# NVlabs/FoundationPose

Hardware: NVIDIA H100
Metric: pose-hypotheses/sec at 640x480 RGB-D, 252 hyp, 5 refine iters (higher is better)
Workload: dtype f16

## Files before the change

### foundationpose_b200/csrc/fp_api_ops.cu

```cuda
#include "../../include/fpose.h"
#include "fp_common.cuh"
#include "fp_attn.cuh"
#include "fp_crop.cuh"
#include "fp_gemm.cuh"

#include <vector>

namespace fp {
const char* get_last_error();
int prof_collect(int kind, double* total_ms, double* total_work, int* launches);
}

extern "C" {

const char* fp_last_error(void) { return fp::get_last_error(); }

unsigned long long fp_launch_count(void) { return fp::launch_count(); }

int fp_prof_enable(int on) {
  fp::g_prof_on = on != 0;
  return 0;
}

int fp_prof_collect(int kind, double* total_ms, double* total_work, int* launches) {
  if (!total_ms || !total_work || !launches) {
    fp::set_last_error("fp_prof_collect: null output");
    return -1;
  }
  return fp::prof_collect(kind, total_ms, total_work, launches);
}

int fp_op_build_meshlets(int V, int F, const float* pos, const int* faces, int* info, int* face_of_tri_out,
                         float* meshlets_out) {
  try {
    if (!pos || !faces || !info || V <= 0 || F <= 0) {
      fp::set_last_error("fp_op_build_meshlets: bad argument");
      return -1;
    }
    for (int i = 0; i < 3 * F; ++i)
      if (faces[i] < 0 || faces[i] >= V) {
        fp::set_last_error("fp_op_build_meshlets: face index out of range");
        return -1;
      }
    std::vector<float> nrm((size_t)V * 3, 0.f), att((size_t)V * 3, 0.f);
    fp::MeshHost mh;
    int rc = fp::build_mesh_host(V, F, pos, nrm.data(), att.data(), 3, faces, mh);
    if (rc) return rc;
    int max_t = 0, max_v = 0, total = 0;
    for (const fp::Meshlet& m : mh.meshlets) {
      max_t = m.n_tris > max_t ? m.n_tris : max_t;
      max_v = m.n_verts > max_v ? m.n_verts : max_v;
      total += m.n_tris;
      for (int t = 0; t < m.n_tris; ++t) {
        const uint2 tr = mh.ml_tris[m.tri_off + t];
        for (int k = 0; k < 3; ++k) {
          const int slot = (tr.x >> (8 * k)) & 255;
          if (slot >= m.n_verts || mh.ml_verts[m.vert_off + slot] != faces[3 * tr.y + k]) {
            fp::set_last_error("fp_op_build_meshlets: meshlet triangle does not map back to its face");
            return -4;
          }
          const float* q = pos + 3 * faces[3 * tr.y + k];
          const float dx = q[0] - m.cx, dy = q[1] - m.cy, dz = q[2] - m.cz;
          if (dx * dx + dy * dy + dz * dz > m.r * m.r * 1.0001f + 1e-12f) {
            fp::set_last_error("fp_op_build_meshlets: vertex outside the meshlet's bounding sphere");
            return -4;
          }
        }
        if (face_of_tri_out) face_of_tri_out[m.tri_off + t] = (int)tr.y;
      }
    }
    if (meshlets_out)
      for (size_t i = 0; i < mh.meshlets.size(); ++i) {
        const fp::Meshlet& m = mh.meshlets[i];
        const float rec[8] = {m.cx, m.cy, m.cz, m.r, m.ax, m.ay, m.az, m.cutoff};
        for (int k = 0; k < 8; ++k) meshlets_out[8 * i + k] = rec[k];
      }
    info[0] = (int)mh.meshlets.size();
    info[1] = mh.closed;
    info[2] = mh.front_sign;
    info[3] = max_t;
    info[4] = max_v;
    info[5] = total;
    return 0;
  } catch (...) {
    fp::set_last_error("fp_op_build_meshlets: exception");
    return -3;
  }
}

int fp_op_attention(const void* qkv, void* out, int B, int impl, void* stream) {
  if (!qkv || !out) {
    fp::set_last_error("fp_op_attention: null argument");
    return -1;
  }
  fp::AttnParams ap;
  ap.qkv = reinterpret_cast<const __half*>(qkv);
  ap.ld = 1536;
  ap.q_off = 0;
  ap.k_off = 512;
  ap.v_off = 1024;
  ap.group_col_stride = 0;
  ap.n_groups = 1;
  ap.out = reinterpret_cast<__half*>(out);
  ap.ld_out = 512;
  ap.out_group_stride = 0;
  ap.B = B;
  ap.T = 400;
  ap.n_heads = 4;
  ap.scale = 0.08838834764831845f;
  cudaStream_t st = reinterpret_cast<cudaStream_t>(stream);
  (void)impl;
  return fp::attn_tc_launch(ap, st);
}

static fp::GemmLayer to_gemm_layer(const fp_gemm_layer_t* l) {
  fp::GemmLayer L;
  L.kind = l->kind;
  L.n_img = l->n_img;
  L.Hin = l->Hin;
  L.Win = l->Win;
  L.Cin = l->Cin;
  L.Cout = l->Cout;
  L.in = l->in;
  L.w = l->w;
  L.bias = l->bias;
  L.res = l->res;
  L.res_ld = l->res_ld;
  L.out = l->out;
  L.out_ld = l->out_ld;
  L.out_split = l->out_split;
  L.post_add = l->post_add;
  L.relu = l->relu;
  return L;
}

int fp_op_gemm_layer(const fp_gemm_layer_t* l, void* stream) {
  if (!l) {
    fp::set_last_error("fp_op_gemm_layer: null layer");
    return -1;
  }
  return fp::gemm_layer_launch(to_gemm_layer(l), reinterpret_cast<cudaStream_t>(stream));
}

int fp_op_gemm_tile_n(const fp_gemm_layer_t* l, int* tile_n) {
  if (!l || !tile_n) {
    fp::set_last_error("fp_op_gemm_tile_n: null argument");
    return -1;
  }
  return fp::gemm_layer_tile_n(to_gemm_layer(l), tile_n);
}

}
```

### foundationpose_b200/csrc/fp_gemm.cu

```cuda
#include "fp_gemm.cuh"

#include <stdarg.h>
#include <stdlib.h>
#include <string.h>

#include <mutex>
#include <vector>

#include "fp_common.cuh"
#include "fp_wgmma.cuh"

namespace fp {

static std::atomic<unsigned long long> g_launch_count{0};
static thread_local bool t_capturing = false;
void note_launches(int n) {
  if (!t_capturing) g_launch_count.fetch_add((unsigned long long)n, std::memory_order_relaxed);
}
unsigned long long launch_count() { return g_launch_count.load(std::memory_order_relaxed); }
void set_capturing(bool on) { t_capturing = on; }

std::atomic<bool> g_prof_on{false};
static std::mutex g_prof_mu;

struct ProfRec {
  cudaEvent_t e0, e1;
  double work;
  int kind;
};
static std::vector<ProfRec> g_prof_recs;

void prof_mark_begin(int kind, double work, cudaStream_t stream) {
  if (!g_prof_on) return;
  ProfRec r;
  r.kind = kind;
  r.work = work;
  cudaEventCreate(&r.e0);
  cudaEventCreate(&r.e1);
  cudaEventRecord(r.e0, stream);
  std::lock_guard<std::mutex> lk(g_prof_mu);
  g_prof_recs.push_back(r);
}
void prof_mark_end(cudaStream_t stream) {
  if (!g_prof_on) return;
  std::lock_guard<std::mutex> lk(g_prof_mu);
  if (g_prof_recs.empty()) return;
  cudaEventRecord(g_prof_recs.back().e1, stream);
}
int prof_collect(int kind, double* total_ms, double* total_work, int* launches) {
  FP_CUDA_OK(cudaDeviceSynchronize());
  std::lock_guard<std::mutex> lk(g_prof_mu);
  double ms = 0, work = 0;
  int n = 0;
  std::vector<ProfRec> keep;
  for (auto& r : g_prof_recs) {
    if (r.kind != kind) {
      keep.push_back(r);
      continue;
    }
    float t = 0.f;
    cudaEventElapsedTime(&t, r.e0, r.e1);
    ms += t;
    work += r.work;
    ++n;
    cudaEventDestroy(r.e0);
    cudaEventDestroy(r.e1);
  }
  g_prof_recs.swap(keep);
  *total_ms = ms;
  *total_work = work;
  *launches = n;
  return 0;
}

static thread_local char t_last_error[1024] = "";
void set_last_error(const char* fmt, ...) {
  va_list ap;
  va_start(ap, fmt);
  vsnprintf(t_last_error, sizeof(t_last_error), fmt, ap);
  va_end(ap);
}
const char* get_last_error() { return t_last_error; }

static thread_local int t_pdl_skip = 0;
void pdl_skip_next() { t_pdl_skip = 1; }

bool pdl_enabled() {
  if (t_pdl_skip) {
    t_pdl_skip = 0;
    return false;
  }
  static int on = -1;
  if (on < 0) {
    const char* e = getenv("FPOSE_PDL");
    on = (e && e[0] == '0') ? 0 : 1;
  }
  return on != 0;
}

struct GemmParams {
  int lg_bw, lg_bh;
  int bw, bh, bn;
  int tiles_w, tiles_h, tiles_n, n_tiles_n, total_tiles;
  int num_kb, chunks_per_tap;
  int dim_w, dim_h, dim_n;
  short tap_off[9][5];
  int Ho, Wo, n_img, Cout;
  const float* bias;
  int has_res;
  int odim_h, odim_n;
  int out_split;
  const float* post_add;
  int relu;
  double alg_flops;
};

constexpr int kBlockM = 128;
constexpr int kBlockK = 64;
constexpr int kABytes = kBlockM * kBlockK * 2;
constexpr int kTileThreads = 384;
constexpr int kSlabBytes = kBlockM * 64 * 2;
constexpr int kSmemOptIn = 232448;

constexpr int kWideSlabs = 2;
constexpr int kWideProducerRegs = 40;
constexpr int kWideConsumerRegs = 232;
template <int BN>
struct TileCfg {
  static constexpr int kBBytes = BN * kBlockK * 2;
  static constexpr int kStageBytes = kABytes + kBBytes;
  static constexpr int kSlabs = BN > 128 ? kWideSlabs : BN / 64;
  static constexpr int kPasses = BN / 64 / kSlabs;
  static constexpr int kStagingBytes = kSlabs * kSlabBytes;
  static constexpr int kRing = kSmemOptIn - kStagingBytes - 1024  - 256 ;
  static constexpr int kStages = (kRing / kStageBytes) > 8 ? 8 : (kRing / kStageBytes);
  static constexpr int kSmemBytes = kStages * kStageBytes + kStagingBytes + 1024 + 256;
  static_assert(kSmemBytes <= kSmemOptIn, "tile configuration exceeds the 227 KB opt-in shared memory");
  static_assert(kPasses * kSlabs * 64 == BN, "the epilogue passes must cover the tile's channels");
};

template <int BN>
__global__ void __launch_bounds__(kTileThreads, 1)
    gemm_tile_kernel(const __grid_constant__ CUtensorMap map_a, const __grid_constant__ CUtensorMap map_b,
                     const __grid_constant__ CUtensorMap map_out, const __grid_constant__ CUtensorMap map_res,
                     const __grid_constant__ GemmParams p) {
  using Cfg = TileCfg<BN>;
  constexpr int S = Cfg::kStages;
  constexpr int NSLAB = Cfg::kSlabs;
  constexpr int JP = BN / 8 / Cfg::kPasses;
  extern __shared__ uint8_t smem_raw[];
  uint8_t* smem = reinterpret_cast<uint8_t*>((reinterpret_cast<uintptr_t>(smem_raw) + 1023) & ~uintptr_t(1023));
  uint8_t* staging = smem + S * Cfg::kStageBytes;
  uint64_t* bars = reinterpret_cast<uint64_t*>(staging + Cfg::kStagingBytes);
  uint64_t* full = bars;
  uint64_t* empty = bars + S;
  uint64_t* res_full = bars + 2 * S;

  const int m_tiles = p.tiles_w * p.tiles_h * p.tiles_n;
  const int total = m_tiles * p.n_tiles_n;

  if (threadIdx.x == 0) {
    tma_prefetch_desc(&map_a);
    tma_prefetch_desc(&map_b);
    tma_prefetch_desc(&map_out);
    if (p.has_res) tma_prefetch_desc(&map_res);
    for (int s = 0; s < S; ++s) {
      mbar_init(&full[s], 1);
      mbar_init(&empty[s], 256);
    }
    mbar_init(res_full, 1);
    mbar_fence_init();
  }
  __syncthreads();
  pdl_trigger();
  pdl_wait();

  auto decode = [&](int t, int& n_tile, int& tw, int& th, int& tn) {
    n_tile = t % p.n_tiles_n;
    const int m_tile = t / p.n_tiles_n;
    tw = m_tile % p.tiles_w;
    th = (m_tile / p.tiles_w) % p.tiles_h;
    tn = m_tile / (p.tiles_w * p.tiles_h);
  };

  if (threadIdx.x < 128) {
    if constexpr (BN > 128) regs_release<kWideProducerRegs>();
    if (threadIdx.x == 0) {
      int stage = 0, phase = 0;
      for (int t = blockIdx.x; t < total; t += gridDim.x) {
        int n_tile, tw, th, tn;
        decode(t, n_tile, tw, th, tn);
        int base[5] = {0, 0, 0, 0, 0};
        base[p.dim_w] += tw * p.bw;
        if (p.dim_h >= 0) base[p.dim_h] += th * p.bh;
        if (p.dim_n >= 0) base[p.dim_n] += tn * p.bn;
        int tap = 0, chunk = 0;
        for (int kb = 0; kb < p.num_kb; ++kb) {
          mbar_wait(&empty[stage], phase ^ 1);
          uint8_t* sa = smem + stage * Cfg::kStageBytes;
          mbar_expect_tx(&full[stage], Cfg::kStageBytes);
          tma_load_5d(&map_a, &full[stage], sa, base[0] + p.tap_off[tap][0] + chunk * kBlockK, base[1] + p.tap_off[tap][1],
                      base[2] + p.tap_off[tap][2], base[3] + p.tap_off[tap][3], base[4] + p.tap_off[tap][4]);
          tma_load_2d(&map_b, &full[stage], sa + kABytes, kb * kBlockK, n_tile * BN);
          if (++chunk == p.chunks_per_tap) {
            chunk = 0;
            ++tap;
          }
          if (++stage == S) {
            stage = 0;
            phase ^= 1;
          }
        }
      }
    }
    return;
  }

  if constexpr (BN > 128) regs_acquire<kWideConsumerRegs>();
  const int ct = threadIdx.x - 128;
  const int cw = ct >> 7;
  const int lane = threadIdx.x & 31;
  const int r0 = 64 * cw + 16 * ((ct >> 5) & 3) + (lane >> 2);
  const int cq = 2 * (lane & 3);
  const bool leader = (ct == 0);
  float acc[BN / 2];
#pragma unroll
  for (int i = 0; i < BN / 2; ++i) acc[i] = 0.f;
  int stage = 0, phase = 0, it = 0;
  for (int t = blockIdx.x; t < total; t += gridDim.x, ++it) {
    int n_tile, tw, th, tn;
    decode(t, n_tile, tw, th, tn);
    const int n0 = tn * p.bn;
    int n_o0 = n0, coff = 0;
    if (p.out_split > 0) {
      n_o0 = n0 % p.out_split;
      coff = (n0 / p.out_split) * p.Cout;
    }
    int oc[5] = {0, 0, 0, 0, 0}, rc[5] = {0, 0, 0, 0, 0};
    oc[1] = rc[1] = tw * p.bw;
    if (p.odim_h >= 0) oc[p.odim_h] = rc[p.odim_h] = th * p.bh;
    if (p.odim_n >= 0) {
      oc[p.odim_n] = n_o0;
      rc[p.odim_n] = n0;
    }
    if (leader) asm volatile("cp.async.bulk.wait_group.read 0;" ::: "memory");
    asm volatile("bar.sync 1, 256;" ::: "memory");
    if (leader && p.has_res) {
      mbar_expect_tx(res_full, NSLAB * kSlabBytes);
      for (int s = 0; s < NSLAB; ++s)
        tma_load_5d(&map_res, res_full, staging + s * kSlabBytes, n_tile * BN + s * 64, rc[1], rc[2], rc[3], rc[4]);
    }

    int prev = -1;
    for (int kb = 0; kb < p.num_kb; ++kb) {
      mbar_wait(&full[stage], phase);
      const uint32_t sa = smem_u32(smem + stage * Cfg::kStageBytes);
      const uint64_t da = gmma_desc_sw128(sa + (uint32_t)cw * 8192u);
      const uint64_t db = gmma_desc_sw128(sa + kABytes);
      wgmma_fence();
#pragma unroll
      for (int k = 0; k < kBlockK / 16; ++k)
        Wgmma<BN>::ss(acc, da + (uint64_t)(2 * k), db + (uint64_t)(2 * k), (kb > 0 || k > 0) ? 1u : 0u);
      wgmma_commit();
      if (prev >= 0) {
        wgmma_wait<1>();
        mbar_arrive(&empty[prev]);
      }
      prev = stage;
      if (++stage == S) {
        stage = 0;
        phase ^= 1;
      }
    }
    wgmma_wait<0>();
    fence_regs(acc);
    if (prev >= 0) mbar_arrive(&empty[prev]);

    const float* bias = p.bias + n_tile * BN;
    const float* pap[2] = {nullptr, nullptr};
    if (p.post_add) {
#pragma unroll
      for (int h = 0; h < 2; ++h) {
        const int row = r0 + 8 * h;
        const int jj = row & (p.bw - 1), ii = (row >> p.lg_bw) & (p.bh - 1);
        const int i = th * p.bh + ii, j = min(tw * p.bw + jj, p.Wo - 1);
        pap[h] = p.post_add + (size_t)(i * p.Wo + j) * p.Cout + n_tile * BN;
      }
    }
#pragma unroll
    for (int ps = 0; ps < Cfg::kPasses; ++ps) {
      const int c0 = n_tile * BN + ps * NSLAB * 64;
      if (ps > 0) {
        if (leader) asm volatile("cp.async.bulk.wait_group.read 0;" ::: "memory");
        asm volatile("bar.sync 1, 256;" ::: "memory");
        if (leader && p.has_res) {
          mbar_expect_tx(res_full, NSLAB * kSlabBytes);
          for (int s = 0; s < NSLAB; ++s)
            tma_load_5d(&map_res, res_full, staging + s * kSlabBytes, c0 + s * 64, rc[1], rc[2], rc[3], rc[4]);
        }
      }
      if (p.has_res) mbar_wait(res_full, (uint32_t)((it * Cfg::kPasses + ps) & 1));
#pragma unroll
      for (int jl = 0; jl < JP; ++jl) {
        const int j = ps * JP + jl;
        const int col = 8 * j + cq;
        const float2 b = __ldg(reinterpret_cast<const float2*>(bias + col));
        uint8_t* slab = staging + (jl >> 3) * kSlabBytes;
#pragma unroll
        for (int h = 0; h < 2; ++h) {
          const int row = r0 + 8 * h;
          uint32_t* cell = reinterpret_cast<uint32_t*>(slab + row * 128 + ((((uint32_t)j & 7u) ^ (uint32_t)(row & 7)) << 4) + cq * 2);
          float a0 = acc[4 * j + 2 * h] + b.x, a1 = acc[4 * j + 2 * h + 1] + b.y;
          if (p.has_res) {
            const float2 r = __half22float2(*reinterpret_cast<const __half2*>(cell));
            a0 += r.x;
            a1 += r.y;
          }
          if (p.relu) {
            a0 = fmaxf(a0, 0.f);
            a1 = fmaxf(a1, 0.f);
          }
          if (pap[h]) {
            const float2 pe = __ldg(reinterpret_cast<const float2*>(pap[h] + col));
            a0 += pe.x;
            a1 += pe.y;
          }
          *cell = pack_half2(a0, a1);
        }
      }
      asm volatile("fence.proxy.async.shared::cta;" ::: "memory");
      asm volatile("bar.sync 1, 256;" ::: "memory");
      if (leader) {
        for (int s = 0; s < NSLAB; ++s)
          tma_store_5d(&map_out, staging + s * kSlabBytes, coff + c0 + s * 64, oc[1], oc[2], oc[3], oc[4]);
        asm volatile("cp.async.bulk.commit_group;" ::: "memory");
      }
    }
  }
  if (leader) asm volatile("cp.async.bulk.wait_group 0;" ::: "memory");
}

static int g_num_sms = 0;

typedef CUresult (*EncodeTiledFn)(CUtensorMap*, CUtensorMapDataType, cuuint32_t, void*, const cuuint64_t*,
                                  const cuuint64_t*, const cuuint32_t*, const cuuint32_t*,
                                  CUtensorMapInterleave, CUtensorMapSwizzle, CUtensorMapL2promotion,
                                  CUtensorMapFloatOOBfill);

static EncodeTiledFn get_encode_fn() {
  static EncodeTiledFn fn = nullptr;
  static std::once_flag once;
  std::call_once(once, [] {
    void* p = nullptr;
    cudaDriverEntryPointQueryResult qres;
    if (cudaGetDriverEntryPoint("cuTensorMapEncodeTiled", &p, cudaEnableDefault, &qres) == cudaSuccess &&
        qres == cudaDriverEntryPointSuccess)
      fn = reinterpret_cast<EncodeTiledFn>(p);
  });
  return fn;
}

static int encode_map(CUtensorMap* map, const void* base, int rank, const uint64_t* dims,
                      const uint64_t* strides_bytes , const uint32_t* box, bool swizzle128 = true) {
  EncodeTiledFn fn = get_encode_fn();
  FP_REQUIRE(fn != nullptr, "cuTensorMapEncodeTiled entry point not available (no CUDA driver?)");
  cuuint64_t gdim[5];
  cuuint64_t gstr[4];
  cuuint32_t bdim[5];
  cuuint32_t estr[5];
  for (int i = 0; i < rank; ++i) {
    gdim[i] = dims[i];
    bdim[i] = box[i];
    estr[i] = 1;
  }
  for (int i = 0; i < rank - 1; ++i) gstr[i] = strides_bytes[i];
  CUresult r = fn(map, CU_TENSOR_MAP_DATA_TYPE_FLOAT16, (cuuint32_t)rank, const_cast<void*>(base), gdim, gstr,
                  bdim, estr, CU_TENSOR_MAP_INTERLEAVE_NONE, swizzle128 ? CU_TENSOR_MAP_SWIZZLE_128B : CU_TENSOR_MAP_SWIZZLE_NONE,
                  CU_TENSOR_MAP_L2_PROMOTION_L2_256B, CU_TENSOR_MAP_FLOAT_OOB_FILL_NONE);
  FP_REQUIRE(r == CUDA_SUCCESS,
             "cuTensorMapEncodeTiled failed (%d): rank %d dims [%llu %llu %llu %llu %llu] box [%u %u %u %u %u]",
             (int)r, rank, (unsigned long long)dims[0], (unsigned long long)(rank > 1 ? dims[1] : 0),
             (unsigned long long)(rank > 2 ? dims[2] : 0), (unsigned long long)(rank > 3 ? dims[3] : 0),
             (unsigned long long)(rank > 4 ? dims[4] : 0), box[0], rank > 1 ? box[1] : 0, rank > 2 ? box[2] : 0,
             rank > 3 ? box[3] : 0, rank > 4 ? box[4] : 0);
  return 0;
}

int encode_map_f16(CUtensorMap* map, const void* base, int rank, const uint64_t* dims, const uint64_t* strides_bytes,
                   const uint32_t* box) {
  return encode_map(map, base, rank, dims, strides_bytes, box);
}
int encode_map_f16_linear(CUtensorMap* map, const void* base, int rank, const uint64_t* dims,
                          const uint64_t* strides_bytes, const uint32_t* box) {
  return encode_map(map, base, rank, dims, strides_bytes, box, false);
}
int num_sms() {
  if (g_num_sms == 0) {
    int dev = 0;
    if (cudaGetDevice(&dev) != cudaSuccess) return 0;
    if (cudaDeviceGetAttribute(&g_num_sms, cudaDevAttrMultiProcessorCount, dev) != cudaSuccess) return 0;
  }
  return g_num_sms;
}

static int ilog2(int v) {
  int l = 0;
  while ((1 << l) < v) ++l;
  return l;
}

template <int BN>
static int launch_bn(const CUtensorMap& ma, const CUtensorMap& mb, const CUtensorMap& mo, const CUtensorMap& mr,
                     const GemmParams& p, cudaStream_t stream) {
  using Cfg = TileCfg<BN>;
  static std::atomic<unsigned long long> attr_mask{0};
  if (!device_bit_test(attr_mask)) {
    FP_CUDA_OK(cudaFuncSetAttribute(gemm_tile_kernel<BN>, cudaFuncAttributeMaxDynamicSharedMemorySize, Cfg::kSmemBytes));
    device_bit_set(attr_mask);
  }
  const int sms = num_sms();
  FP_REQUIRE(sms > 0, "no CUDA device");
  const int grid = p.total_tiles < sms ? p.total_tiles : sms;
  prof_mark_begin(0, p.alg_flops, stream);
  FP_CUDA_OK(launch_pdl(gemm_tile_kernel<BN>, dim3(grid), dim3(kTileThreads), Cfg::kSmemBytes, stream, 1, ma, mb, mo, mr, p));
  prof_mark_end(stream);
  note_launches(1);
  FP_CUDA_OK(cudaGetLastError());
  return 0;
}

int stem_conv_launch(const GemmLayer& L, cudaStream_t stream);

static int gemm_layer_plan(const GemmLayer& L, cudaStream_t stream, int* tile_n) {
  if (L.kind == LK_CONV7_S2) {
    if (tile_n) {
      *tile_n = 64;
      return 0;
    }
    return stem_conv_launch(L, stream);
  }
  GemmParams p;
  memset(&p, 0, sizeof(p));
  CUtensorMap ma, mb;
  const uint64_t E = 2;
  int Ho, Wo, taps, ktot;
  int BN;
  uint64_t dims[5], str[4];
  uint32_t box[5];

  switch (L.kind) {
    case LK_LINEAR: {
      FP_REQUIRE(L.Cin % 64 == 0, "LINEAR: K=%d not a multiple of 64", L.Cin);
      Ho = 1;
      Wo = L.Win;
      taps = 1;
      p.chunks_per_tap = L.Cin / 64;
      p.bw = 128; p.bh = 1; p.bn = 1;
      p.dim_w = 1; p.dim_h = -1; p.dim_n = -1;
      dims[0] = L.Cin; dims[1] = L.Win; dims[2] = 1; dims[3] = 1; dims[4] = 1;
      str[0] = L.Cin * E; str[1] = str[0] * L.Win; str[2] = str[1]; str[3] = str[1];
      box[0] = 64; box[1] = 128; box[2] = 1; box[3] = 1; box[4] = 1;
      p.tiles_w = (L.Win + 127) / 128; p.tiles_h = 1; p.tiles_n = 1;
      break;
    }
    case LK_CONV3_S1: {
      FP_REQUIRE(L.Cin % 64 == 0, "CONV3_S1: Cin=%d not a multiple of 64", L.Cin);
      Ho = L.Hin; Wo = L.Win;
      taps = 9;
      p.chunks_per_tap = L.Cin / 64;
      if (Wo % 8 == 0 && Ho % 8 == 0) { p.bw = 8; p.bh = 8; p.bn = 2; }
      else if (Wo % 4 == 0 && Ho % 4 == 0) { p.bw = 4; p.bh = 4; p.bn = 8; }
      else FP_REQUIRE(false, "CONV3_S1: unsupported spatial size %dx%d", Ho, Wo);
      const uint64_t sw_ = (uint64_t)L.Cin * E, sh_ = sw_ * L.Win, sn_ = sh_ * L.Hin;
      p.dim_w = 1; p.dim_h = 2; p.dim_n = 3;
      dims[0] = L.Cin; dims[1] = L.Win; dims[2] = L.Hin; dims[3] = L.n_img; dims[4] = 1;
      str[0] = sw_; str[1] = sh_; str[2] = sn_; str[3] = sn_ * L.n_img;
      box[0] = 64; box[1] = p.bw; box[2] = p.bh; box[3] = p.bn; box[4] = 1;
      for (int r = 0; r < 3; ++r)
        for (int s = 0; s < 3; ++s) {
          p.tap_off[r * 3 + s][1] = (short)(s - 1);
          p.tap_off[r * 3 + s][2] = (short)(r - 1);
        }
      p.tiles_w = Wo / p.bw; p.tiles_h = Ho / p.bh; p.tiles_n = (L.n_img + p.bn - 1) / p.bn;
      break;
    }
    case LK_CONV3_S2: {
      FP_REQUIRE(L.Cin % 64 == 0, "CONV3_S2: Cin=%d not a multiple of 64", L.Cin);
      FP_REQUIRE(L.Hin % 2 == 0 && L.Win % 2 == 0, "CONV3_S2: odd input size");
      Ho = L.Hin / 2; Wo = L.Win / 2;
      taps = 9;
      p.chunks_per_tap = L.Cin / 64;
      if (Wo % 8 == 0 && Ho % 8 == 0) { p.bw = 8; p.bh = 8; p.bn = 2; }
      else if (Wo % 4 == 0 && Ho % 4 == 0) { p.bw = 4; p.bh = 4; p.bn = 8; }
      else FP_REQUIRE(false, "CONV3_S2: unsupported output size %dx%d", Ho, Wo);
      p.dim_w = 1; p.dim_h = 3; p.dim_n = 4;
      dims[0] = 2 * L.Cin; dims[1] = Wo; dims[2] = 2; dims[3] = Ho; dims[4] = L.n_img;
      str[0] = 2 * L.Cin * E; str[1] = (uint64_t)L.Win * L.Cin * E; str[2] = 2 * str[1];
      str[3] = (uint64_t)L.Hin * L.Win * L.Cin * E;
      box[0] = 64; box[1] = p.bw; box[2] = 1; box[3] = p.bh; box[4] = p.bn;
      for (int r = 0; r < 3; ++r)
        for (int s = 0; s < 3; ++s) {
          const int t = r * 3 + s;
          p.tap_off[t][0] = (short)((s == 1 ? 0 : 1) * L.Cin);
          p.tap_off[t][1] = (short)(s == 0 ? -1 : 0);
          p.tap_off[t][2] = (short)(r == 1 ? 0 : 1);
          p.tap_off[t][3] = (short)(r == 0 ? -1 : 0);
        }
      p.tiles_w = Wo / p.bw; p.tiles_h = Ho / p.bh; p.tiles_n = (L.n_img + p.bn - 1) / p.bn;
      break;
    }
    default:
      FP_REQUIRE(false, "unknown layer kind %d", L.kind);
  }
  ktot = taps * L.Cin;
  p.num_kb = ktot / 64;
  p.lg_bw = ilog2(p.bw);
  p.lg_bh = ilog2(p.bh);

  constexpr int kWideMinWaves = 8;
  constexpr int kWideMinKBlocks = 16;
  const int m_tiles = p.tiles_w * p.tiles_h * p.tiles_n;
  if (L.Cout % 256 == 0 && p.num_kb >= kWideMinKBlocks) {
    const int sms = num_sms();
    FP_REQUIRE(sms > 0, "no CUDA device");
    BN = (long long)m_tiles * (L.Cout / 256) >= (long long)kWideMinWaves * sms ? 256 : 128;
  } else if (L.Cout % 128 == 0) BN = 128;
  else if (L.Cout % 64 == 0) BN = 64;
  else FP_REQUIRE(false, "Cout=%d must be a multiple of 64", L.Cout);
  p.n_tiles_n = L.Cout / BN;
  p.total_tiles = p.tiles_w * p.tiles_h * p.tiles_n * p.n_tiles_n;
  p.Ho = Ho; p.Wo = Wo; p.n_img = L.n_img; p.Cout = L.Cout;
  p.bias = L.bias;
  p.has_res = L.res != nullptr;
  p.out_split = L.out_split;
  p.post_add = L.post_add;
  p.relu = L.relu;
  {
    const double k_real = (double)taps * L.Cin;
    p.alg_flops = 2.0 * (double)L.n_img * Ho * Wo * L.Cout * k_real;
  }
  FP_REQUIRE(L.out_ld % 8 == 0 && (!L.res || L.res_ld % 8 == 0), "out_ld / res_ld must be multiples of 8");
  FP_REQUIRE(L.out_split == 0 || L.out_split % p.bn == 0,
             "out_split=%d must be a multiple of the tile's image count %d (pad the A/B batch boundary)", L.out_split,
             p.bn);
  if (tile_n) {
    *tile_n = BN;
    return 0;
  }
  if (p.total_tiles == 0) return 0;

  int rc = encode_map(&ma, L.in, 5, dims, str, box);
  if (rc) return rc;
  uint64_t wd[2] = {(uint64_t)ktot, (uint64_t)L.Cout};
  uint64_t ws[1] = {(uint64_t)ktot * E};
  uint32_t wb[2] = {64, (uint32_t)BN};
  rc = encode_map(&mb, L.w, 2, wd, ws, wb);
  if (rc) return rc;
  CUtensorMap mo, mr;
  {
    uint64_t od[5], os[4];
    uint32_t ob[5];
    const bool lin = (L.kind == LK_LINEAR);
    const int n_out = L.out_split > 0 ? (L.n_img - L.out_split) : L.n_img;
    FP_REQUIRE(n_out > 0, "out_split=%d leaves no output images (n_img=%d)", L.out_split, L.n_img);
    auto fill = [&](int ld, int nimg) {
      const uint64_t sw_ = (uint64_t)ld * E, sh_ = sw_ * Wo, sn_ = sh_ * Ho;
      od[0] = (uint64_t)ld;
      ob[0] = 64;
      od[4] = 1;
      ob[4] = 1;
      if (lin) {
        od[1] = (uint64_t)Wo; od[2] = 1; od[3] = 1;
        os[0] = sw_; os[1] = sh_; os[2] = sh_; os[3] = sh_;
        ob[1] = (uint32_t)p.bw; ob[2] = 1; ob[3] = 1;
      } else {
        od[1] = (uint64_t)Wo; od[2] = (uint64_t)Ho; od[3] = (uint64_t)nimg;
        os[0] = sw_; os[1] = sh_; os[2] = sn_; os[3] = sn_ * nimg;
        ob[1] = (uint32_t)p.bw; ob[2] = (uint32_t)p.bh; ob[3] = (uint32_t)p.bn;
      }
    };
    p.odim_h = lin ? -1 : 2;
    p.odim_n = lin ? -1 : 3;
    fill(L.out_ld, n_out);
    rc = encode_map(&mo, L.out, 5, od, os, ob);
    if (rc) return rc;
    if (L.res) {
      fill(L.res_ld, L.n_img);
      rc = encode_map(&mr, L.res, 5, od, os, ob);
      if (rc) return rc;
    } else {
      mr = mo;
    }
  }
  if (BN == 256) return launch_bn<256>(ma, mb, mo, mr, p, stream);
  return BN == 128 ? launch_bn<128>(ma, mb, mo, mr, p, stream) : launch_bn<64>(ma, mb, mo, mr, p, stream);
}

int gemm_layer_launch(const GemmLayer& L, cudaStream_t stream) { return gemm_layer_plan(L, stream, nullptr); }

int gemm_layer_tile_n(const GemmLayer& L, int* tile_n) { return gemm_layer_plan(L, nullptr, tile_n); }

}
```

### foundationpose_b200/csrc/fp_gemm.cuh

```cuda
#pragma once
#include <cuda.h>
#include <cuda_runtime.h>
#include <stdint.h>

#include <atomic>

namespace fp {

enum LayerKind : int {
  LK_LINEAR = 0,
  LK_CONV3_S1 = 1,
  LK_CONV3_S2 = 2,
  LK_CONV7_S2 = 3,
};

struct GemmLayer {
  int kind;
  int n_img;
  int Hin, Win;
  int Cin;
  int Cout;
  const void* in;
  const void* w;
  const float* bias;
  const void* res;
  int res_ld;
  void* out;
  int out_ld;
  int out_split;
  const float* post_add;
  int relu;
};

int gemm_layer_launch(const GemmLayer& L, cudaStream_t stream);
int gemm_layer_tile_n(const GemmLayer& L, int* tile_n);


void prof_mark_begin(int kind, double work, cudaStream_t stream);
void prof_mark_end(cudaStream_t stream);
extern std::atomic<bool> g_prof_on;

}
```

### foundationpose_b200/ops.py

```python
import ctypes as C

import torch

from . import _lib
from ._lib import lib


def _ptr(t):
    return None if t is None else C.c_void_p(t.data_ptr())


def _stream():
    return C.c_void_p(torch.cuda.current_stream().cuda_stream)


def _require_cuda(*ts):
    for t in ts:
        if t is not None and not t.is_cuda:
            raise _lib.FposeError("libfpose operators need CUDA tensors (there is no CPU path)")


def gemm_layer(kind, x, w_packed, bias, *, n_img, Hin, Win, Cin, Cout, out=None, out_ld=None, out_split=0,
               res=None, res_ld=0, post_add=None, relu=False):
    _require_cuda(x, w_packed, bias, res, post_add, out)
    assert x.dtype == torch.float16 and w_packed.dtype == torch.float16 and bias.dtype == torch.float32
    if kind == _lib.LAYER_LINEAR:
        Ho, Wo = 1, Win
    elif kind == _lib.LAYER_CONV3_S1:
        Ho, Wo = Hin, Win
    else:
        Ho, Wo = Hin // 2, Win // 2
    if out is None:
        out_ld = Cout
        out = torch.empty(n_img, Ho, Wo, Cout, dtype=torch.float16, device=x.device)
    L = _lib.GemmLayer(kind, n_img, Hin, Win, Cin, Cout, _ptr(x), _ptr(w_packed), _ptr(bias), _ptr(res),
                       res_ld, _ptr(out), out_ld, out_split, _ptr(post_add), 1 if relu else 0)
    _lib.check(lib.fp_op_gemm_layer(C.byref(L), _stream()), "fp_op_gemm_layer")
    return out


def gemm_tile_n(kind, *, n_img, Hin, Win, Cin, Cout, out_split=0):
    lib.fp_op_gemm_tile_n.argtypes = [C.POINTER(_lib.GemmLayer), C.POINTER(C.c_int)]
    lib.fp_op_gemm_tile_n.restype = C.c_int
    L = _lib.GemmLayer(kind, n_img, Hin, Win, Cin, Cout, None, None, None, None, 0, None, Cout, out_split, None, 0)
    tile_n = C.c_int(0)
    _lib.check(lib.fp_op_gemm_tile_n(C.byref(L), C.byref(tile_n)), "fp_op_gemm_tile_n")
    return tile_n.value


lib.fp_op_attention.argtypes = [C.c_void_p, C.c_void_p, C.c_int, C.c_int, C.c_void_p]
lib.fp_op_attention.restype = C.c_int


def attention(qkv, impl=1):
    _require_cuda(qkv)
    assert qkv.dtype == torch.float16 and qkv.shape[1] == 1536 and qkv.shape[0] % 400 == 0
    B = qkv.shape[0] // 400
    out = torch.empty(qkv.shape[0], 512, dtype=torch.float16, device=qkv.device)
    _lib.check(lib.fp_op_attention(_ptr(qkv), _ptr(out), B, impl, _stream()), "fp_op_attention")
    return out
```

### include/fpose.h

```cpp
#ifndef FPOSE_H_
#define FPOSE_H_

#include <stddef.h>
#include <stdint.h>

#ifdef __cplusplus
extern "C" {
#endif

const char* fp_last_error(void);
unsigned long long fp_launch_count(void);

int fp_prof_enable(int on);
int fp_prof_collect(int kind, double* total_ms, double* total_work, int* launches);


#define FP_LAYER_LINEAR 0
#define FP_LAYER_CONV3_S1 1
#define FP_LAYER_CONV3_S2 2
#define FP_LAYER_CONV7_S2 3

typedef struct fp_gemm_layer {
  int kind;
  int n_img;
  int Hin, Win;
  int Cin;
  int Cout;
  const void* in;
  const void* w;
  const float* bias;
  const void* res;
  int res_ld;
  void* out;
  int out_ld;
  int out_split;
  const float* post_add;
  int relu;
} fp_gemm_layer_t;

int fp_op_gemm_layer(const fp_gemm_layer_t* layer, void* stream);
int fp_op_gemm_tile_n(const fp_gemm_layer_t* layer, int* tile_n);

int fp_op_attention(const void* qkv, void* out, int B, int impl, void* stream);


typedef struct fp_ctx fp_ctx;

int fp_create(fp_ctx** ctx);
int fp_destroy(fp_ctx* ctx);

int fp_set_config(fp_ctx* ctx, int which, float crop_ratio, float rot_normalizer);

typedef struct fp_tensor {
  const char* name;
  const void* data;
  int dtype;
  long long numel;
} fp_tensor_t;

int fp_load_network(fp_ctx* ctx, int which, const fp_tensor_t* tensors, int n);

int fp_set_mesh(fp_ctx* ctx, int V, int F, const float* pos, const float* nrm, const float* uv, const float* vcol,
                const int* faces, const unsigned char* tex_rgb, int Ht, int Wt, float diameter);
#define FP_MAX_MESHES 64
int fp_set_mesh_slot(fp_ctx* ctx, int slot, int V, int F, const float* pos, const float* nrm, const float* uv,
                     const float* vcol, const int* faces, const unsigned char* tex_rgb, int Ht, int Wt, float diameter);
int fp_mesh_info(fp_ctx* ctx, int* info);

#define FP_FRAME_ON_DEVICE 1
#define FP_FRAME_FILTER_DEPTH 2
int fp_set_frame(fp_ctx* ctx, const unsigned char* rgb, const float* depth, const float* K, int H, int W, int flags,
                 float zfar, void* stream);
int fp_set_xyz_map(fp_ctx* ctx, const float* xyz, void* stream);
int fp_get_depth(fp_ctx* ctx, float* depth_out_dev, float* xyz_out_dev, void* stream);

int fp_start_poses(fp_ctx* ctx, const unsigned char* mask, int mask_on_device, const float* rot_grid, int N,
                   float* poses_out, float* info_out, void* stream);

int fp_make_crops(fp_ctx* ctx, const float* poses, int N, int mode, void* crops_out, float* dbg_out, float* win_out,
                  void* stream);
int fp_set_crop_tile(fp_ctx* ctx, int tile);
int fp_crop_stats(fp_ctx* ctx, const float* poses, int N, int mode, int* stats_out_host, void* stream);

int fp_refine(fp_ctx* ctx, const float* poses_in, int N, int iterations, float* poses_out, float* last_trans,
              float* last_rot, void* stream);

int fp_score(fp_ctx* ctx, const float* poses, int N, float* scores_out, int* best_out, void* stream);
int fp_score_features(fp_ctx* ctx, const float* poses, int N, float* feats_out, void* stream);
int fp_score_tail(fp_ctx* ctx, const float* feats, int L, float* scores_out, int* best_out, void* stream);

int fp_register(fp_ctx* ctx, const float* poses_host, int N, int iterations, float* poses_out_host,
                float* scores_out_host, int* best_out_host, void* stream);

int fp_track(fp_ctx* ctx, const unsigned char* rgb_host, const float* depth_host, const float* K, int H, int W,
             const float* pose_in_dev, int iterations, float* pose_out_dev, float* pose_out_host, void* stream);
int fp_track_objects(fp_ctx* ctx, const unsigned char* rgb_host, const float* depth_host, const float* K, int H, int W,
                     int M, const int* slots_host, const float* poses_in_dev, int iterations, float* poses_out_dev,
                     float* poses_out_host, void* stream);
#define FP_MAX_CAMERAS 16
int fp_track_cameras(fp_ctx* ctx, int C, const unsigned char* const* rgb_host, const float* const* depth_host,
                     const float* K, const int* H, const int* W, int M, const int* camera_of, const int* slots_host,
                     const float* poses_in_dev, int iterations, float* poses_out_dev, float* poses_out_host, void* stream);
int fp_register_objects(fp_ctx* ctx, const unsigned char* rgb_host, const float* depth_host, const float* K, int H, int W,
                        int M, const int* slots_host, const int* n_hyp_host, const unsigned char* masks_host,
                        const float* rot_grids_dev, int iterations, float* poses_out_dev, float* scores_out_dev,
                        int* best_out_dev, float* info_out_dev, void* stream);
int fp_register_cameras(fp_ctx* ctx, int C, const unsigned char* const* rgb_host, const float* const* depth_host,
                        const float* K, const int* H, const int* W, int M, const int* camera_of, const int* slots_host,
                        const int* n_hyp_host, const unsigned char* const* masks_host, const float* rot_grids_dev,
                        int iterations, float* poses_out_dev, float* scores_out_dev, int* best_out_dev, float* info_out_dev,
                        void* stream);
unsigned long long fp_graph_captures(fp_ctx* ctx);

typedef struct fp_group fp_group;
int fp_group_create(int ndev, const int* dev_ids, fp_group** out);
int fp_group_destroy(fp_group* g);
int fp_group_size(fp_group* g);
fp_ctx* fp_group_ctx(fp_group* g, int i);
int fp_group_load_network(fp_group* g, int which, const fp_tensor_t* tensors, int n);
int fp_group_set_config(fp_group* g, int which, float crop_ratio, float rot_normalizer);
int fp_group_set_mesh(fp_group* g, int V, int F, const float* pos, const float* nrm, const float* uv, const float* vcol,
                      const int* faces, const unsigned char* tex_rgb, int Ht, int Wt, float diameter);
int fp_group_register(fp_group* g, const unsigned char* rgb_host, const float* depth_host, const float* K, int H, int W,
                      const unsigned char* mask_host, const float* rot_grid_host, int N, int iterations,
                      float* poses_out_host, float* scores_out_host, int* best_out_host, float* info_out_host);

int fp_op_refine_net(fp_ctx* ctx, const void* crops, int N, float* trans_out, float* rot_out, void* stream);
int fp_op_score_feats(fp_ctx* ctx, const void* crops, int N, float* feats_out, void* stream);
int fp_op_tokens(fp_ctx* ctx, int which, const void* crops, int N, void* tokens_out, void* stream);
int fp_op_build_meshlets(int V, int F, const float* pos, const int* faces, int* info, int* face_of_tri_out,
                         float* meshlets_out );
int fp_op_depth_filter(const float* depth_dev, float* out_dev, int H, int W, int which, void* stream);
int fp_op_pose_update(const float* poses_in, const float* trans, const float* rot, float* poses_out, int N,
                      float mesh_diameter, float rot_normalizer, void* stream);

#ifdef __cplusplus
}
#endif
#endif
```

Measured before the change: 2618.

## Add ping-pong warpgroup schedule for 128-wide GEMM tiles with enough waves

Adds a ping-pong variant of the persistent TMA/WGMMA GEMM kernel. Each consumer warpgroup owns a whole 128x128 tile and the two warpgroups alternate mainloop turns via named barriers, so one group's epilogue overlaps the other's tensor-core work. Each group gets its own staging slabs and residual barrier. It is picked automatically for 128-wide layers with at least two waves of tiles, and an API to query or force the schedule is added. In exchange the ring shrinks to 5 stages to make room for the doubled staging buffer, and each consumer holds 128 accumulator registers.

```diff
diff --git a/foundationpose_b200/csrc/fp_api_ops.cu b/foundationpose_b200/csrc/fp_api_ops.cu
--- a/foundationpose_b200/csrc/fp_api_ops.cu
+++ b/foundationpose_b200/csrc/fp_api_ops.cu
@@ -147,7 +147,33 @@
     fp::set_last_error("fp_op_gemm_tile_n: null argument");
     return -1;
   }
-  return fp::gemm_layer_tile_n(to_gemm_layer(l), tile_n);
+  fp::GemmSchedule s;
+  const int rc = fp::gemm_layer_schedule(to_gemm_layer(l), &s);
+  if (rc == 0) *tile_n = s.tile_n;
+  return rc;
+}
+
+int fp_op_gemm_schedule(const fp_gemm_layer_t* l, int* tile_n, int* schedule) {
+  if (!l || !tile_n || !schedule) {
+    fp::set_last_error("fp_op_gemm_schedule: null argument");
+    return -1;
+  }
+  fp::GemmSchedule s;
+  const int rc = fp::gemm_layer_schedule(to_gemm_layer(l), &s);
+  if (rc == 0) {
+    *tile_n = s.tile_n;
+    *schedule = s.schedule;
+  }
+  return rc;
+}
+
+int fp_op_gemm_layer_with(const fp_gemm_layer_t* l, int tile_n, int schedule, void* stream) {
+  if (!l) {
+    fp::set_last_error("fp_op_gemm_layer_with: null layer");
+    return -1;
+  }
+  return fp::gemm_layer_launch_with(to_gemm_layer(l), fp::GemmSchedule{tile_n, schedule},
+                                    reinterpret_cast<cudaStream_t>(stream));
 }
 
 }
diff --git a/foundationpose_b200/csrc/fp_gemm.cu b/foundationpose_b200/csrc/fp_gemm.cu
--- a/foundationpose_b200/csrc/fp_gemm.cu
+++ b/foundationpose_b200/csrc/fp_gemm.cu
@@ -125,26 +125,77 @@
 constexpr int kWideSlabs = 2;
 constexpr int kWideProducerRegs = 40;
 constexpr int kWideConsumerRegs = 232;
-template <int BN>
+enum : int { kCooperative = 0, kPingPong = 1 };
+template <int BN, int kSched = kCooperative>
 struct TileCfg {
   static constexpr int kBBytes = BN * kBlockK * 2;
   static constexpr int kStageBytes = kABytes + kBBytes;
   static constexpr int kSlabs = BN > 128 ? kWideSlabs : BN / 64;
   static constexpr int kPasses = BN / 64 / kSlabs;
-  static constexpr int kStagingBytes = kSlabs * kSlabBytes;
+  static constexpr int kStagingBytes = (kSched == kPingPong ? 2 : 1) * kSlabs * kSlabBytes;
   static constexpr int kRing = kSmemOptIn - kStagingBytes - 1024  - 256 ;
   static constexpr int kStages = (kRing / kStageBytes) > 8 ? 8 : (kRing / kStageBytes);
   static constexpr int kSmemBytes = kStages * kStageBytes + kStagingBytes + 1024 + 256;
   static_assert(kSmemBytes <= kSmemOptIn, "tile configuration exceeds the 227 KB opt-in shared memory");
   static_assert(kPasses * kSlabs * 64 == BN, "the epilogue passes must cover the tile's channels");
+  static_assert(kSched == kCooperative || BN == 128, "ping-pong runs 128 x 128 tiles only (one per warpgroup)");
+  static_assert(kSched != kPingPong || kStages == 5, "ping-pong: 5 ring stages of 32 KB + 4 staging slabs of 16 KB");
 };
 
-template <int BN>
+template <int JP, int N>
+__device__ __forceinline__ void epilogue_pass(const float (&acc)[N], int j0, uint32_t staging, int r0, int cq,
+                                              const float* bias, const float* const (&pap)[2], bool has_res, bool relu) {
+#pragma unroll
+  for (int jl = 0; jl < JP; ++jl) {
+    const int j = j0 + jl;
+    const int col = 8 * j + cq;
+    const float2 b = __ldg(reinterpret_cast<const float2*>(bias + col));
+    const uint32_t slab = staging + (uint32_t)(jl >> 3) * kSlabBytes;
+#pragma unroll
+    for (int h = 0; h < 2; ++h) {
+      const int row = r0 + 8 * h;
+      const uint32_t cell = slab + row * 128 + ((((uint32_t)j & 7u) ^ (uint32_t)(row & 7)) << 4) + cq * 2;
+      float a0 = acc[4 * j + 2 * h] + b.x, a1 = acc[4 * j + 2 * h + 1] + b.y;
+      if (has_res) {
+        uint32_t rv;
+        asm volatile("ld.shared.b32 %0, [%1];" : "=r"(rv) : "r"(cell));
+        const float2 r = __half22float2(*reinterpret_cast<const __half2*>(&rv));
+        a0 += r.x;
+        a1 += r.y;
+      }
+      if (relu) {
+        a0 = fmaxf(a0, 0.f);
+        a1 = fmaxf(a1, 0.f);
+      }
+      if (pap[h]) {
+        const float2 pe = __ldg(reinterpret_cast<const float2*>(pap[h] + col));
+        a0 += pe.x;
+        a1 += pe.y;
+      }
+      asm volatile("st.shared.b32 [%0], %1;" ::"r"(cell), "r"(pack_half2(a0, a1)));
+    }
+  }
+}
+
+__device__ __forceinline__ void pe_rows(const GemmParams& p, int r0, int tw, int th, int c0, const float* (&pap)[2]) {
+#pragma unroll
+  for (int h = 0; h < 2; ++h) {
+    pap[h] = nullptr;
+    if (p.post_add) {
+      const int row = r0 + 8 * h;
+      const int jj = row & (p.bw - 1), ii = (row >> p.lg_bw) & (p.bh - 1);
+      const int i = th * p.bh + ii, j = min(tw * p.bw + jj, p.Wo - 1);
+      pap[h] = p.post_add + (size_t)(i * p.Wo + j) * p.Cout + c0;
+    }
+  }
+}
+
+template <int BN, int kSched = kCooperative>
 __global__ void __launch_bounds__(kTileThreads, 1)
     gemm_tile_kernel(const __grid_constant__ CUtensorMap map_a, const __grid_constant__ CUtensorMap map_b,
                      const __grid_constant__ CUtensorMap map_out, const __grid_constant__ CUtensorMap map_res,
                      const __grid_constant__ GemmParams p) {
-  using Cfg = TileCfg<BN>;
+  using Cfg = TileCfg<BN, kSched>;
   constexpr int S = Cfg::kStages;
   constexpr int NSLAB = Cfg::kSlabs;
   constexpr int JP = BN / 8 / Cfg::kPasses;
@@ -166,9 +217,10 @@
     if (p.has_res) tma_prefetch_desc(&map_res);
     for (int s = 0; s < S; ++s) {
       mbar_init(&full[s], 1);
-      mbar_init(&empty[s], 256);
+      mbar_init(&empty[s], kSched == kPingPong ? 128 : 256);
     }
     mbar_init(res_full, 1);
+    if constexpr (kSched == kPingPong) mbar_init(res_full + 1, 1);
     mbar_fence_init();
   }
   __syncthreads();
@@ -184,7 +236,7 @@
   };
 
   if (threadIdx.x < 128) {
-    if constexpr (BN > 128) regs_release<kWideProducerRegs>();
+    if constexpr (BN > 128 || kSched == kPingPong) regs_release<kWideProducerRegs>();
     if (threadIdx.x == 0) {
       int stage = 0, phase = 0;
       for (int t = blockIdx.x; t < total; t += gridDim.x) {
@@ -216,33 +268,122 @@
     return;
   }
 
-  if constexpr (BN > 128) regs_acquire<kWideConsumerRegs>();
   const int ct = threadIdx.x - 128;
   const int cw = ct >> 7;
   const int lane = threadIdx.x & 31;
+  const int cq = 2 * (lane & 3);
+  auto tile_boxes = [&](int t, int& n_tile, int& tw, int& th, int (&oc)[5], int (&rc)[5], int& coff) {
+    int tn;
+    decode(t, n_tile, tw, th, tn);
+    const int n0 = tn * p.bn;
+    int n_o0 = n0;
+    coff = 0;
+    if (p.out_split > 0) {
+      n_o0 = n0 % p.out_split;
+      coff = (n0 / p.out_split) * p.Cout;
+    }
+    oc[1] = rc[1] = tw * p.bw;
+    if (p.odim_h >= 0) oc[p.odim_h] = rc[p.odim_h] = th * p.bh;
+    if (p.odim_n >= 0) {
+      oc[p.odim_n] = n_o0;
+      rc[p.odim_n] = n0;
+    }
+  };
+
+  if constexpr (kSched == kPingPong) {
+    regs_acquire<kWideConsumerRegs>();
+    const int r0 = 16 * ((ct >> 5) & 3) + (lane >> 2);
+    const bool leader = (ct & 127) == 0;
+    uint8_t* slabs = staging + cw * NSLAB * kSlabBytes;
+    uint64_t* res_bar = res_full + cw;
+    const uint32_t bar_epi = 2 + cw;
+    const uint32_t bar_turn = 4 + cw, bar_next = 5 - cw;
+    float acc[2][64];
+    int stage = 0, phase = 0;
+    auto skip = [&](int n) {
+      stage += n;
+      const int wraps = stage / S;
+      stage -= wraps * S;
+      phase ^= wraps & 1;
+    };
+    if (cw == 1) {
+      skip(p.num_kb);
+      asm volatile("bar.arrive 4, 256;" ::: "memory");
+    }
+    int it = 0;
+    for (int t = blockIdx.x + cw * gridDim.x; t < total; t += 2 * gridDim.x, ++it) {
+      int n_tile, tw, th, coff;
+      int oc[5] = {0, 0, 0, 0, 0}, rc[5] = {0, 0, 0, 0, 0};
+      tile_boxes(t, n_tile, tw, th, oc, rc, coff);
+      if (leader) asm volatile("cp.async.bulk.wait_group.read 0;" ::: "memory");
+      asm volatile("bar.sync %0, 128;" ::"r"(bar_epi) : "memory");
+      if (leader && p.has_res) {
+        mbar_expect_tx(res_bar, NSLAB * kSlabBytes);
+        for (int s = 0; s < NSLAB; ++s)
+          tma_load_5d(&map_res, res_bar, slabs + s * kSlabBytes, n_tile * BN + s * 64, rc[1], rc[2], rc[3], rc[4]);
+      }
+
+      asm volatile("bar.sync %0, 256;" ::"r"(bar_turn) : "memory");
+      int prev = -1;
+      for (int kb = 0; kb < p.num_kb; ++kb) {
+        mbar_wait(&full[stage], phase);
+        const uint32_t sa = smem_u32(smem + stage * Cfg::kStageBytes);
+        const uint64_t da0 = gmma_desc_sw128(sa);
+        const uint64_t da1 = gmma_desc_sw128(sa + 8192u);
+        const uint64_t db = gmma_desc_sw128(sa + kABytes);
+        wgmma_fence();
+#pragma unroll
+        for (int k = 0; k < kBlockK / 16; ++k) {
+          const uint32_t scale_d = (kb > 0 || k > 0) ? 1u : 0u;
+          Wgmma<BN>::ss(acc[0], da0 + (uint64_t)(2 * k), db + (uint64_t)(2 * k), scale_d);
+          Wgmma<BN>::ss(acc[1], da1 + (uint64_t)(2 * k), db + (uint64_t)(2 * k), scale_d);
+        }
+        wgmma_commit();
+        if (prev >= 0) {
+          wgmma_wait<1>();
+          mbar_arrive(&empty[prev]);
+        }
+        prev = stage;
+        skip(1);
+      }
+      if (t + (int)gridDim.x < total) asm volatile("bar.arrive %0, 256;" ::"r"(bar_next) : "memory");
+      wgmma_wait<0>();
+      fence_regs(acc[0]);
+      fence_regs(acc[1]);
+      if (prev >= 0) mbar_arrive(&empty[prev]);
+      skip(p.num_kb);
+
+      const float* bias = p.bias + n_tile * BN;
+      if (p.has_res) mbar_wait(res_bar, (uint32_t)(it & 1));
+#pragma unroll
+      for (int half = 0; half < 2; ++half) {
+        const float* pap[2];
+        pe_rows(p, r0 + 64 * half, tw, th, n_tile * BN, pap);
+        epilogue_pass<BN / 8>(acc[half], 0, smem_u32(slabs), r0 + 64 * half, cq, bias, pap, p.has_res, p.relu);
+      }
+      asm volatile("fence.proxy.async.shared::cta;" ::: "memory");
+      asm volatile("bar.sync %0, 128;" ::"r"(bar_epi) : "memory");
+      if (leader) {
+        for (int s = 0; s < NSLAB; ++s)
+          tma_store_5d(&map_out, slabs + s * kSlabBytes, coff + n_tile * BN + s * 64, oc[1], oc[2], oc[3], oc[4]);
+        asm volatile("cp.async.bulk.commit_group;" ::: "memory");
+      }
+    }
+    if (leader) asm volatile("cp.async.bulk.wait_group 0;" ::: "memory");
+    return;
+  }
+
+  if constexpr (BN > 128) regs_acquire<kWideConsumerRegs>();
   const int r0 = 64 * cw + 16 * ((ct >> 5) & 3) + (lane >> 2);
-  const int cq = 2 * (lane & 3);
   const bool leader = (ct == 0);
   float acc[BN / 2];
 #pragma unroll
   for (int i = 0; i < BN / 2; ++i) acc[i] = 0.f;
   int stage = 0, phase = 0, it = 0;
   for (int t = blockIdx.x; t < total; t += gridDim.x, ++it) {
-    int n_tile, tw, th, tn;
-    decode(t, n_tile, tw, th, tn);
-    const int n0 = tn * p.bn;
-    int n_o0 = n0, coff = 0;
-    if (p.out_split > 0) {
-      n_o0 = n0 % p.out_split;
-      coff = (n0 / p.out_split) * p.Cout;
-    }
+    int n_tile, tw, th, coff;
     int oc[5] = {0, 0, 0, 0, 0}, rc[5] = {0, 0, 0, 0, 0};
-    oc[1] = rc[1] = tw * p.bw;
-    if (p.odim_h >= 0) oc[p.odim_h] = rc[p.odim_h] = th * p.bh;
-    if (p.odim_n >= 0) {
-      oc[p.odim_n] = n_o0;
-      rc[p.odim_n] = n0;
-    }
+    tile_boxes(t, n_tile, tw, th, oc, rc, coff);
     if (leader) asm volatile("cp.async.bulk.wait_group.read 0;" ::: "memory");
     asm volatile("bar.sync 1, 256;" ::: "memory");
     if (leader && p.has_res) {
@@ -277,16 +418,8 @@
     if (prev >= 0) mbar_arrive(&empty[prev]);
 
     const float* bias = p.bias + n_tile * BN;
-    const float* pap[2] = {nullptr, nullptr};
-    if (p.post_add) {
-#pragma unroll
-      for (int h = 0; h < 2; ++h) {
-        const int row = r0 + 8 * h;
-        const int jj = row & (p.bw - 1), ii = (row >> p.lg_bw) & (p.bh - 1);
-        const int i = th * p.bh + ii, j = min(tw * p.bw + jj, p.Wo - 1);
-        pap[h] = p.post_add + (size_t)(i * p.Wo + j) * p.Cout + n_tile * BN;
-      }
-    }
+    const float* pap[2];
+    pe_rows(p, r0, tw, th, n_tile * BN, pap);
 #pragma unroll
     for (int ps = 0; ps < Cfg::kPasses; ++ps) {
       const int c0 = n_tile * BN + ps * NSLAB * 64;
@@ -300,34 +433,7 @@
         }
       }
       if (p.has_res) mbar_wait(res_full, (uint32_t)((it * Cfg::kPasses + ps) & 1));
-#pragma unroll
-      for (int jl = 0; jl < JP; ++jl) {
-        const int j = ps * JP + jl;
-        const int col = 8 * j + cq;
-        const float2 b = __ldg(reinterpret_cast<const float2*>(bias + col));
-        uint8_t* slab = staging + (jl >> 3) * kSlabBytes;
-#pragma unroll
-        for (int h = 0; h < 2; ++h) {
-          const int row = r0 + 8 * h;
-          uint32_t* cell = reinterpret_cast<uint32_t*>(slab + row * 128 + ((((uint32_t)j & 7u) ^ (uint32_t)(row & 7)) << 4) + cq * 2);
-          float a0 = acc[4 * j + 2 * h] + b.x, a1 = acc[4 * j + 2 * h + 1] + b.y;
-          if (p.has_res) {
-            const float2 r = __half22float2(*reinterpret_cast<const __half2*>(cell));
-            a0 += r.x;
-            a1 += r.y;
-          }
-          if (p.relu) {
-            a0 = fmaxf(a0, 0.f);
-            a1 = fmaxf(a1, 0.f);
-          }
-          if (pap[h]) {
-            const float2 pe = __ldg(reinterpret_cast<const float2*>(pap[h] + col));
-            a0 += pe.x;
-            a1 += pe.y;
-          }
-          *cell = pack_half2(a0, a1);
-        }
-      }
+      epilogue_pass<JP>(acc, ps * JP, smem_u32(staging), r0, cq, bias, pap, p.has_res, p.relu);
       asm volatile("fence.proxy.async.shared::cta;" ::: "memory");
       asm volatile("bar.sync 1, 256;" ::: "memory");
       if (leader) {
@@ -409,20 +515,21 @@
   return l;
 }
 
-template <int BN>
+template <int BN, int kSched = kCooperative>
 static int launch_bn(const CUtensorMap& ma, const CUtensorMap& mb, const CUtensorMap& mo, const CUtensorMap& mr,
                      const GemmParams& p, cudaStream_t stream) {
-  using Cfg = TileCfg<BN>;
+  using Cfg = TileCfg<BN, kSched>;
+  auto kernel = gemm_tile_kernel<BN, kSched>;
   static std::atomic<unsigned long long> attr_mask{0};
   if (!device_bit_test(attr_mask)) {
-    FP_CUDA_OK(cudaFuncSetAttribute(gemm_tile_kernel<BN>, cudaFuncAttributeMaxDynamicSharedMemorySize, Cfg::kSmemBytes));
+    FP_CUDA_OK(cudaFuncSetAttribute(kernel, cudaFuncAttributeMaxDynamicSharedMemorySize, Cfg::kSmemBytes));
     device_bit_set(attr_mask);
   }
   const int sms = num_sms();
   FP_REQUIRE(sms > 0, "no CUDA device");
   const int grid = p.total_tiles < sms ? p.total_tiles : sms;
   prof_mark_begin(0, p.alg_flops, stream);
-  FP_CUDA_OK(launch_pdl(gemm_tile_kernel<BN>, dim3(grid), dim3(kTileThreads), Cfg::kSmemBytes, stream, 1, ma, mb, mo, mr, p));
+  FP_CUDA_OK(launch_pdl(kernel, dim3(grid), dim3(kTileThreads), Cfg::kSmemBytes, stream, 1, ma, mb, mo, mr, p));
   prof_mark_end(stream);
   note_launches(1);
   FP_CUDA_OK(cudaGetLastError());
@@ -431,10 +538,11 @@
 
 int stem_conv_launch(const GemmLayer& L, cudaStream_t stream);
 
-static int gemm_layer_plan(const GemmLayer& L, cudaStream_t stream, int* tile_n) {
+static int gemm_layer_plan(const GemmLayer& L, cudaStream_t stream, const GemmSchedule* force, GemmSchedule* query) {
   if (L.kind == LK_CONV7_S2) {
-    if (tile_n) {
-      *tile_n = 64;
+    FP_REQUIRE(!force || (force->tile_n == 64 && force->schedule == kCooperative), "the 7x7 stem runs 64-wide tiles only");
+    if (query) {
+      *query = GemmSchedule{64, 0};
       return 0;
     }
     return stem_conv_launch(L, stream);
@@ -445,6 +553,7 @@
   const uint64_t E = 2;
   int Ho, Wo, taps, ktot;
   int BN;
+  int sched;
   uint64_t dims[5], str[4];
   uint32_t box[5];
 
@@ -519,6 +628,7 @@
 
   constexpr int kWideMinWaves = 8;
   constexpr int kWideMinKBlocks = 16;
+  constexpr int kPingPongMinWaves = 2;
   const int m_tiles = p.tiles_w * p.tiles_h * p.tiles_n;
   if (L.Cout % 256 == 0 && p.num_kb >= kWideMinKBlocks) {
     const int sms = num_sms();
@@ -527,6 +637,22 @@
   } else if (L.Cout % 128 == 0) BN = 128;
   else if (L.Cout % 64 == 0) BN = 64;
   else FP_REQUIRE(false, "Cout=%d must be a multiple of 64", L.Cout);
+  sched = kCooperative;
+  if (BN == 128) {
+    const int sms = num_sms();
+    FP_REQUIRE(sms > 0, "no CUDA device");
+    if ((long long)m_tiles * (L.Cout / 128) >= (long long)kPingPongMinWaves * sms) sched = kPingPong;
+  }
+  if (force) {
+    FP_REQUIRE((force->tile_n == 64 || force->tile_n == 128 || force->tile_n == 256) && L.Cout % force->tile_n == 0,
+               "no %d-wide tile for Cout=%d", force->tile_n, L.Cout);
+    FP_REQUIRE(force->schedule == kCooperative || force->schedule == kPingPong, "unknown schedule %d",
+               force->schedule);
+    FP_REQUIRE(force->schedule == kCooperative || force->tile_n == 128, "ping-pong runs 128-wide tiles only (asked for %d)",
+               force->tile_n);
+    BN = force->tile_n;
+    sched = force->schedule;
+  }
   p.n_tiles_n = L.Cout / BN;
   p.total_tiles = p.tiles_w * p.tiles_h * p.tiles_n * p.n_tiles_n;
   p.Ho = Ho; p.Wo = Wo; p.n_img = L.n_img; p.Cout = L.Cout;
@@ -543,8 +669,8 @@
   FP_REQUIRE(L.out_split == 0 || L.out_split % p.bn == 0,
              "out_split=%d must be a multiple of the tile's image count %d (pad the A/B batch boundary)", L.out_split,
              p.bn);
-  if (tile_n) {
-    *tile_n = BN;
+  if (query) {
+    *query = GemmSchedule{BN, sched};
     return 0;
   }
   if (p.total_tiles == 0) return 0;
@@ -593,11 +719,16 @@
     }
   }
   if (BN == 256) return launch_bn<256>(ma, mb, mo, mr, p, stream);
+  if (sched == kPingPong) return launch_bn<128, kPingPong>(ma, mb, mo, mr, p, stream);
   return BN == 128 ? launch_bn<128>(ma, mb, mo, mr, p, stream) : launch_bn<64>(ma, mb, mo, mr, p, stream);
 }
 
-int gemm_layer_launch(const GemmLayer& L, cudaStream_t stream) { return gemm_layer_plan(L, stream, nullptr); }
-
-int gemm_layer_tile_n(const GemmLayer& L, int* tile_n) { return gemm_layer_plan(L, nullptr, tile_n); }
-
-}
+int gemm_layer_launch(const GemmLayer& L, cudaStream_t stream) { return gemm_layer_plan(L, stream, nullptr, nullptr); }
+
+int gemm_layer_launch_with(const GemmLayer& L, const GemmSchedule& s, cudaStream_t stream) {
+  return gemm_layer_plan(L, stream, &s, nullptr);
+}
+
+int gemm_layer_schedule(const GemmLayer& L, GemmSchedule* s) { return gemm_layer_plan(L, nullptr, nullptr, s); }
+
+}
diff --git a/foundationpose_b200/csrc/fp_gemm.cuh b/foundationpose_b200/csrc/fp_gemm.cuh
--- a/foundationpose_b200/csrc/fp_gemm.cuh
+++ b/foundationpose_b200/csrc/fp_gemm.cuh
@@ -32,8 +32,15 @@
   int relu;
 };
 
+struct GemmSchedule {
+  int tile_n;
+  int schedule;
+
+};
+
 int gemm_layer_launch(const GemmLayer& L, cudaStream_t stream);
-int gemm_layer_tile_n(const GemmLayer& L, int* tile_n);
+int gemm_layer_launch_with(const GemmLayer& L, const GemmSchedule& s, cudaStream_t stream);
+int gemm_layer_schedule(const GemmLayer& L, GemmSchedule* s);
 
 
 void prof_mark_begin(int kind, double work, cudaStream_t stream);
diff --git a/foundationpose_b200/ops.py b/foundationpose_b200/ops.py
--- a/foundationpose_b200/ops.py
+++ b/foundationpose_b200/ops.py
@@ -21,7 +21,7 @@
 
 
 def gemm_layer(kind, x, w_packed, bias, *, n_img, Hin, Win, Cin, Cout, out=None, out_ld=None, out_split=0,
-               res=None, res_ld=0, post_add=None, relu=False):
+               res=None, res_ld=0, post_add=None, relu=False, schedule=None):
     _require_cuda(x, w_packed, bias, res, post_add, out)
     assert x.dtype == torch.float16 and w_packed.dtype == torch.float16 and bias.dtype == torch.float32
     if kind == _lib.LAYER_LINEAR:
@@ -35,7 +35,14 @@
         out = torch.empty(n_img, Ho, Wo, Cout, dtype=torch.float16, device=x.device)
     L = _lib.GemmLayer(kind, n_img, Hin, Win, Cin, Cout, _ptr(x), _ptr(w_packed), _ptr(bias), _ptr(res),
                        res_ld, _ptr(out), out_ld, out_split, _ptr(post_add), 1 if relu else 0)
-    _lib.check(lib.fp_op_gemm_layer(C.byref(L), _stream()), "fp_op_gemm_layer")
+    if schedule is None:
+        _lib.check(lib.fp_op_gemm_layer(C.byref(L), _stream()), "fp_op_gemm_layer")
+    else:
+        lib.fp_op_gemm_layer_with.argtypes = [C.POINTER(_lib.GemmLayer), C.c_int, C.c_int, C.c_void_p]
+        lib.fp_op_gemm_layer_with.restype = C.c_int
+        tile_n, sched = schedule
+        _lib.check(lib.fp_op_gemm_layer_with(C.byref(L), int(tile_n), int(sched), _stream()),
+                   "fp_op_gemm_layer_with")
     return out
 
 
@@ -46,6 +53,18 @@
     tile_n = C.c_int(0)
     _lib.check(lib.fp_op_gemm_tile_n(C.byref(L), C.byref(tile_n)), "fp_op_gemm_tile_n")
     return tile_n.value
+
+
+GEMM_COOPERATIVE, GEMM_PINGPONG = 0, 1
+
+
+def gemm_schedule(kind, *, n_img, Hin, Win, Cin, Cout, out_split=0):
+    lib.fp_op_gemm_schedule.argtypes = [C.POINTER(_lib.GemmLayer), C.POINTER(C.c_int), C.POINTER(C.c_int)]
+    lib.fp_op_gemm_schedule.restype = C.c_int
+    L = _lib.GemmLayer(kind, n_img, Hin, Win, Cin, Cout, None, None, None, None, 0, None, Cout, out_split, None, 0)
+    tile_n, sched = C.c_int(0), C.c_int(0)
+    _lib.check(lib.fp_op_gemm_schedule(C.byref(L), C.byref(tile_n), C.byref(sched)), "fp_op_gemm_schedule")
+    return tile_n.value, sched.value
 
 
 lib.fp_op_attention.argtypes = [C.c_void_p, C.c_void_p, C.c_int, C.c_int, C.c_void_p]
diff --git a/include/fpose.h b/include/fpose.h
--- a/include/fpose.h
+++ b/include/fpose.h
@@ -40,6 +40,10 @@
 
 int fp_op_gemm_layer(const fp_gemm_layer_t* layer, void* stream);
 int fp_op_gemm_tile_n(const fp_gemm_layer_t* layer, int* tile_n);
+#define FP_GEMM_COOPERATIVE 0
+#define FP_GEMM_PINGPONG 1
+int fp_op_gemm_schedule(const fp_gemm_layer_t* layer, int* tile_n, int* schedule);
+int fp_op_gemm_layer_with(const fp_gemm_layer_t* layer, int tile_n, int schedule, void* stream);
 
 int fp_op_attention(const void* qkv, void* out, int B, int impl, void* stream);
 
```

After: 2683, median of 6. +2.5%, better.
